# cantwellc/QEC_LDPC

Measured on AMD Instinct MI355X. Metric: syndromes decoded/sec (fixed BP iters), higher is better.
Workload: dtype f32

## Files before the change

### include/qec_ldpc.h

```cpp
#ifndef QEC_LDPC_H
#define QEC_LDPC_H

#include <stddef.h>
#include <stdint.h>

#ifdef __cplusplus
extern "C" {
#endif

#define QEC_LDPC_ABI_VERSION 4

enum {
    QEC_OK = 0,
    QEC_ERR_ARG = -1,
    QEC_ERR_IO = -2,
    QEC_ERR_FORMAT = -3,
    QEC_ERR_UNSUPPORTED = -4,
    QEC_ERR_HIP = -5,
    QEC_ERR_NOMEM = -6
};

enum {
    QEC_SUCCESS = 0,
    QEC_SYNDROME_FAIL_X = 1 << 0,
// ... 62 lines not shown

qec_decoder* qec_decoder_create(const qec_code* code, int device, size_t max_batch);
qec_decoder* qec_decoder_create_engine(const qec_code* code, int device, size_t max_batch, int engine);
int qec_decoder_destroy(qec_decoder* dec);
qec_decoder* qec_decoder_create_multi(const qec_code* code, const int* devices, int ndevices, size_t max_batch);
qec_decoder* qec_decoder_create_multi_engine(const qec_code* code, const int* devices, int ndevices, size_t max_batch,
                                             int engine);
int qec_decoder_num_parts(const qec_decoder* dec);
qec_decoder* qec_decoder_part(qec_decoder* dec, int k);
int qec_decoder_device(const qec_decoder* dec);
enum { QEC_OPT_HARD_PATHS = 1, QEC_OPT_CYCLE_JUMP = 2, QEC_OPT_SCHEDULE = 3, QEC_OPT_SECTOR_SPLIT = 4,
       QEC_OPT_PHASE_STATS = 5, QEC_OPT_TRIAGE = 6, QEC_OPT_LAST_PATH = 7, QEC_OPT_MC_DECODE_TIME = 8,
       QEC_OPT_OSD = 9, QEC_OPT_OSD_ITERATIONS = 10, QEC_OPT_OSD_SECTORS = 11, QEC_OPT_OSD_SWEEP = 12,
       QEC_OPT_OSD_ORDER = 13, QEC_OPT_OSD_CS_SECTORS = 14, QEC_OPT_NEAR_HARD_JUMP = 15, QEC_OPT_OSD_SCORE = 16,
       QEC_OPT_CORRELATED = 17, QEC_OPT_BP_SCHEDULE = 18, QEC_OPT_BP_METHOD = 19, QEC_OPT_MINSUM_SCALE = 20,
       QEC_OPT_MINSUM_WAVE = 21, QEC_OPT_RELAY_WAVE = 22, QEC_OPT_MINSUM_SCHEDULE = 23, QEC_OPT_LIGHT_MEMO = 24 };
enum {
    QEC_PATH_ORDERED = 1,
    QEC_PATH_SECTOR_ORDER = 2,
    QEC_PATH_SPLIT_WAVES = 4,
    QEC_PATH_SECTOR_LAUNCHES = 8,
    QEC_PATH_TRIAGE = 16,
    QEC_PATH_BIT_ROWS = 32,
    QEC_PATH_SPARSE = 64,
    QEC_PATH_RECORDS = 128,
    QEC_PATH_OSD = 256,
    QEC_PATH_CORRELATED = 512,
    QEC_PATH_SERIAL = 1024,
    QEC_PATH_MINSUM = 2048,
    QEC_PATH_RELAY = 4096,
    QEC_PATH_SOFT = 16384,
    QEC_PATH_WAVE = 8192
};
int qec_near_hard_threshold(float pPrime, int R, int L, float* eps0, uint32_t* T);
int qec_decoder_set_option(qec_decoder* dec, int option, int value);
int qec_decoder_get_option(const qec_decoder* dec, int option, int* value);
int qec_decoder_set_priors(qec_decoder* dec, const float* priorX, const float* priorZ);
int qec_decoder_get_priors(const qec_decoder* dec, float* priorX, float* priorZ);
int qec_decoder_get_osd_weights(const qec_decoder* dec, int32_t* wX, int32_t* wZ);
int qec_minsum_llr(float prior, float* llr);
int qec_decoder_get_minsum_llr(const qec_decoder* dec, float* llrX, float* llrZ);
int qec_decoder_set_relay(qec_decoder* dec, const float* gammaX, const float* gammaZ, int legs, int solutions);
int qec_decoder_get_relay(const qec_decoder* dec, float* gammaX, float* gammaZ, int* legs, int* solutions);
int qec_decoder_set_syndrome_priors(qec_decoder* dec, const float* qX, const float* qZ);
int qec_decoder_get_syndrome_priors(const qec_decoder* dec, float* qX, float* qZ);
int qec_correlated_priors(float p, float* c0, float* c1);
int qec_decoder_set_pauli_channel(qec_decoder* dec, const float* pX, const float* pY, const float* pZ);
int qec_decoder_get_pauli_channel(const qec_decoder* dec, float* pX, float* pY, float* pZ);
int qec_decoder_get_conditional_priors(const qec_decoder* dec, float* cZ0, float* cZ1, float* cX0, float* cX1);
// ... 76 lines not shown
```

### qec_ldpc_amd/__init__.py

```python
import ctypes
import os

import numpy as np

_HERE = os.path.dirname(os.path.abspath(__file__))
LIB_PATH = os.path.join(_HERE, "libqecldpc.so")

SUCCESS = 0
SYNDROME_FAIL_X = 1
SYNDROME_FAIL_Z = 2
CONVERGENCE_FAIL_X = 4
CONVERGENCE_FAIL_Z = 8
STOP = {"ref": 0, "fixed": 1, "syndrome": 2}
ENGINE = {"auto": 0, "circulant": 1, "sparse": 2, "cpu": 3}
OPTION = {"hard_paths": 1, "cycle_jump": 2, "schedule": 3, "sector_split": 4, "phase_stats": 5, "triage": 6,
          "last_path": 7, "mc_decode_time": 8, "osd": 9, "osd_iterations": 10, "osd_sectors": 11,
          "osd_sweep": 12, "osd_order": 13, "osd_cs_sectors": 14, "near_hard": 15, "osd_score": 16,
          "correlated": 17, "bp_schedule": 18, "bp_method": 19, "minsum_scale": 20,
          "minsum_wave": 21, "relay_wave": 22, "minsum_schedule": 23, "light_memo": 24}
OPTIONS = OPTION
BP_SCHEDULE = {"flooding": 0, "serial": 1}
BP_METHOD = {"product": 0, "minsum": 1}
MINSUM_SCHEDULE = {"flooding": 0, "layered": 1}
PATH = {"ordered": 1, "sector_order": 2, "split_waves": 4, "sector_launches": 8, "triage": 16, "bit_rows": 32,
        "sparse": 64, "records": 128, "osd": 256, "correlated": 512, "serial": 1024,
        "minsum": 2048, "relay": 4096, "wave": 8192, "soft": 16384}

EXPORTS = (
    "qec_last_error", "qec_abi_version", "qec_build_id",
    "qec_code_load", "qec_code_generate", "qec_code_from_matrices", "qec_code_degrees", "qec_code_layers",
    "qec_code_has_wave_minsum",
    "qec_code_free",
    "qec_code_params", "qec_code_exponents",
    "qec_code_pcm", "qec_code_describe", "qec_code_syndrome", "qec_code_check_logical",
    "qec_code_with_logical", "qec_code_logical_mode", "qec_code_logical_rows", "qec_code_imp",
    "qec_decoder_create", "qec_decoder_create_engine", "qec_decoder_create_multi", "qec_decoder_create_multi_engine",
    "qec_decoder_destroy",
    "qec_decoder_num_parts", "qec_decoder_part", "qec_decoder_device", "qec_decoder_describe",
    "qec_decoder_set_option", "qec_decoder_get_option", "qec_near_hard_threshold",
    "qec_decoder_set_priors", "qec_decoder_get_priors", "qec_decoder_get_osd_weights", "qec_sample_independent_dev",
    "qec_correlated_priors", "qec_minsum_llr", "qec_decoder_get_minsum_llr", "qec_decoder_set_pauli_channel", "qec_decoder_get_pauli_channel",
    "qec_decoder_set_relay", "qec_decoder_get_relay",
    "qec_decoder_set_syndrome_priors", "qec_decoder_get_syndrome_priors",
    "qec_decode_batch_soft", "qec_decode_batch_soft_dev", "qec_flip_syndrome_dev",
    "qec_decoder_get_conditional_priors", "qec_sample_pauli_dev",
    "qec_decode_batch", "qec_decode_batch_dev", "qec_decode_batch_packed", "qec_decode_batch_packed_dev",
    "qec_decode_bits_packed_dev",
    "qec_sample_fixed_weight", "qec_get_statistics",
    "qec_sample_depolarizing_dev", "qec_sample_syndrome_dev", "qec_syndrome_dev", "qec_statistics_dev",
    "qec_statistics_packed_dev", "qec_logical_packed_dev", "qec_pack_decisions_dev",
    "qec_monte_carlo",
    "qec_osd", "qec_osd_dev",
)
LOGICAL = {"file": 0, "reference": 1, "degenerate": 2}
# ... 67 lines not shown
            "qec_code_logical_mode": (i, [vp]),
            "qec_code_logical_rows": (i, [vp, vp]),
            "qec_code_imp": (i, [vp, vp]),
            "qec_decoder_create": (vp, [vp, i, sz]),
            "qec_decoder_create_engine": (vp, [vp, i, sz, i]),
            "qec_decoder_create_multi": (vp, [vp, vp, i, sz]),
            "qec_decoder_create_multi_engine": (vp, [vp, vp, i, sz, i]),
            "qec_decoder_destroy": (i, [vp]),
            "qec_decoder_num_parts": (i, [vp]),
            "qec_decoder_part": (vp, [vp, i]),
            "qec_decoder_device": (i, [vp]),
            "qec_decoder_describe": (i, [vp, ctypes.c_char_p, sz]),
            "qec_decoder_set_option": (i, [vp, i, i]),
            "qec_decoder_get_option": (i, [vp, i, vp]),
            "qec_near_hard_threshold": (i, [f, i, i, vp, vp]),
            "qec_decoder_set_priors": (i, [vp, vp, vp]),
            "qec_decoder_get_priors": (i, [vp, vp, vp]),
            "qec_decoder_get_osd_weights": (i, [vp, vp, vp]),
            "qec_sample_independent_dev": (i, [vp, ctypes.c_uint64, ctypes.c_uint64, sz, vp, vp, vp]),
            "qec_correlated_priors": (i, [f, vp, vp]),
            "qec_minsum_llr": (i, [f, vp]),
            "qec_decoder_get_minsum_llr": (i, [vp, vp, vp]),
            "qec_decoder_set_relay": (i, [vp, vp, vp, i, i]),
            "qec_decoder_get_relay": (i, [vp, vp, vp, vp, vp]),
            "qec_decoder_set_syndrome_priors": (i, [vp, vp, vp]),
            "qec_decoder_get_syndrome_priors": (i, [vp, vp, vp]),
            "qec_decode_batch_soft": (i, [vp, vp, vp, sz, f, i, i, vp, vp, vp, vp, vp, vp, vp]),
            "qec_decode_batch_soft_dev": (i, [vp, vp, vp, sz, f, i, i, vp, vp, vp, vp, vp, vp, vp, vp]),
            "qec_flip_syndrome_dev": (i, [vp, ctypes.c_uint64, ctypes.c_uint64, sz, vp, vp, vp, vp, vp]),
            "qec_decoder_set_pauli_channel": (i, [vp, vp, vp, vp]),
# ... 30 lines not shown
def last_error():
    return lib().qec_last_error().decode()


def build_id():
    return lib().qec_build_id().decode()


def near_hard_threshold(p_prime, R, L):
    eps0, T = ctypes.c_float(0.0), ctypes.c_uint32(0)
    _check(lib().qec_near_hard_threshold(float(np.float32(p_prime)), int(R), int(L), ctypes.byref(eps0), ctypes.byref(T)),
           "qec_near_hard_threshold")
    return float(eps0.value), int(T.value)


def correlated_priors(p):
    c0, c1 = ctypes.c_float(0.0), ctypes.c_float(0.0)
    _check(lib().qec_correlated_priors(float(np.float32(p)), ctypes.byref(c0), ctypes.byref(c1)), "qec_correlated_priors")
    return np.float32(c0.value), np.float32(c1.value)


def has_wave_minsum(code):
    return code.has_wave_minsum()


def minsum_llr(prior):
    llr = ctypes.c_float(0.0)
    _check(lib().qec_minsum_llr(float(np.float32(prior)), ctypes.byref(llr)), "qec_minsum_llr")
    return np.float32(llr.value)

# ... 682 lines not shown
```

### qec_ldpc_amd/csrc/bp_decode.hip

```cpp
#include <hip/hip_runtime.h>

#include <atomic>
#include <cstddef>
#include <cstdint>
#include <cstdio>
#include <cstdlib>
#include <cstring>
#include <type_traits>

#include "qec_device.h"
#include "qec_internal.h"
#include "qec_launch.h"
#include "qec_near.h"
#include "qec_wave.h"

#pragma clang fp contract(off)

namespace qec {

#ifndef QEC_PHASE_STATS
#define QEC_PHASE_STATS 0
#endif
constexpr int kTrackFrom = 2;

// ... 4 lines not shown
    static constexpr int kMinWavesX = MWX_ > 0 ? MWX_ : MINW_;
    static constexpr int kMinWavesZ = MWZ_ > 0 ? MWZ_ : MINW_;
    static constexpr bool kRowBarrier = ROWB_;
    static constexpr int kColGroup = CG_;
    static constexpr int kMinWaves = MINW_;
    static constexpr int kMinWavesSyn = SYNW_ > 0 ? SYNW_ : MINW_;
    static constexpr int kWavesPerBlock = WPB_;
    static constexpr bool kMaskSelect = MASKSEL_;
    static constexpr int kPipeline = PIPE_;
    static constexpr bool kSplit = SPLIT_;
    static constexpr bool kRelabel = RELABEL_;
    static constexpr bool kZeroSkip = ZEROSKIP_;
    static constexpr bool kFastDiv = FASTDIV_;
    static constexpr bool kSaturate = SATURATE_;
    static constexpr bool kAgreeSyn = false;
    static constexpr int kSeqSynWavesX = kMinWavesSyn, kSeqSynWavesZ = kMinWavesSyn;
};

template <class TU>
struct SeqSynTune : TU {
    static constexpr int kSeqSynWavesX = 5 > TU::kMinWavesSyn ? 5 : TU::kMinWavesSyn;
};

template <class TU, int LW, int WPB = 0>
struct ListTune : TU {
    static constexpr int kMinWavesSyn = LW;
    static constexpr int kWavesPerBlock = WPB > 0 ? WPB : TU::kWavesPerBlock;
};

template <class TU, int L>
// ... 57 lines not shown
    uint8_t* rec;
    uint32_t* merge;
    const int32_t* listX;
    const int32_t* listZ;
    const uint32_t* counts;
    int mergeOnly;
    int countStride;
    long long B;
    int P, G, n, mX, mZ;
    int nb, recBytes;
    float errorProbability;
    int maxIter, stop;
    int hardPaths;
    int scaled;
    uint32_t nearT[2];
    alignas(16) float tab0[kMaxTab0];
    uint32_t zs[2];
    const uint16_t* memo;
    int SX[kMaxRL], SZ[kMaxRL];
    int DX[kMaxR], DZ[kMaxR];
    int CX[kMaxL], CZ[kMaxL];
};

struct RuntimeShifts {
    static constexpr bool kStatic = false;
    static constexpr bool kMaskSelect = false;
    static constexpr int kP = 0;
    __device__ static int P(const BpArgs& a) { return a.P; }
    template <int SEC>
    __device__ static const int* table(const BpArgs& a)
// ... 246 lines not shown
        for (int r = 0; r < R; ++r) {
            const int sh = SH::template shift<SEC, L>(et, r, l);
            msg[r][l] = rot<SH>(msg[r][l], ln, sh == 0 ? 0 : P - sh);
        }
}

template <int SEC>
__device__ __forceinline__ uint32_t near_T(const BpArgs&)
{
    static_assert(std::is_standard_layout<BpArgs>::value, "offsetof(BpArgs, nearT)");
    const __attribute__((address_space(4))) uint32_t* k =
        (const __attribute__((address_space(4))) uint32_t*)__builtin_amdgcn_kernarg_segment_ptr();
    asm volatile("" : "+s"(k));
    return k[offsetof(BpArgs, nearT) / sizeof(uint32_t) + SEC];
}

template <int R, int L, int SEC, bool LAST, bool HD, class SH, class TU, int CG = 1, bool SOFT_IN = false,
          bool NEAR = false>
__device__ __forceinline__ uint32_t var_pass(const BpArgs& a, float (&msg)[R][L], const Lane& ln, float pp,
                                             float one_minus_pp, bool& hard, bool& vagree, bool track, bool& near)
{
    static_assert(L % CG == 0, "column groups must tile the L columns");
    const bool hard_in = !SOFT_IN && CG == 1 && hard;
    bool vsame = true;
    uint32_t soft_bits = 0;
    constexpr int F = LAST ? R : R - 1;
    constexpr bool kScalable = TU::kFastDiv && F <= 4;
    const bool scaled = kScalable && a.scaled;
    const float fold0 = scaled ? one_minus_pp * 0x1p32f : one_minus_pp, fold1 = scaled ? pp * 0x1p32f : pp;
    const int P = SH::P(a);
// ... 144 lines not shown
        }
        __builtin_amdgcn_sched_barrier(0);
    }
    if constexpr (TU::kSaturate) {
        const bool forms = track && (a.hardPaths & QEC_HP_FORMS);
        hard = forms && all_live_sh<SH>(soft_bits == 0u, ln.live);
        vagree = hard && all_live_sh<SH>(vsame, ln.live);
        if constexpr (NEAR) {
            const uint32_t nearT = near_T<SEC>(a);
            near = nearT != 0u && forms && all_live_sh<SH>(soft_bits <= nearT && vsame, ln.live);
        }
    }
    return hdmask;
}

template <int R, int L, int SEC, bool HD, class SH>
__device__ __forceinline__ bool var_pass_agree(const BpArgs& a, const float (&msg)[R][L], const Lane& ln,
                                               uint32_t& hdmask)
{
    const int* et = SH::template table<SEC>(a);
    bool same = true;
    uint32_t hd = 0;
#pragma unroll
    for (int l = 0; l < L; ++l) {
        const uint32_t x0 = __float_as_uint(rot<SH>(msg[0][l], ln, SH::template shift<SEC, L>(et, 0, l)));
#pragma unroll
        for (int r = 1; r < R; ++r)
            same &= __float_as_uint(rot<SH>(msg[r][l], ln, SH::template shift<SEC, L>(et, r, l))) == x0;
        if constexpr (HD) hd |= (uint32_t)(x0 == 0x3F800000u) << l;
    }
// ... 62 lines not shown
template <int SEC, int L, class SH>
constexpr bool kRow0Local()
{
    if constexpr (!SH::kStatic) {
        return false;
    } else {
        for (int l = 0; l < L; ++l)
            if (SH::template shift<SEC, L>(nullptr, 0, l) != 0) return false;
        return true;
    }
}

template <int L>
constexpr bool kSkipSeen() { return L < 32; }

template <int R, int L, int SEC, int STOP, bool LAST, class SH, class TU>
__device__ __forceinline__ bool iteration(const BpArgs& a, float (&msg)[R][L], uint32_t sbits, int n, Lane& ln,
                                          float pp, float one_minus_pp, bool& hard, bool& agreed, bool& vagree,
                                          uint32_t& hd_out, uint32_t (&seen)[2], bool& near)
{
    const int P = SH::P(a);
    if constexpr (SH::kMaskSelect) asm volatile("" : "+v"(ln.b0), "+v"(ln.b1));
    constexpr bool HD = STOP == QEC_STOP_SYNDROME;
    uint32_t hdmask = 0;
    agreed = false;
    vagree = false;
    near = false;
    bool unused = false;
    bool var_layout = defer_return<HD, SH>();
    if (TU::kSaturate && hard) {
        check_pass_hard<R, L>(msg, sbits);
        agreed = kAgree<STOP, TU>() && (LAST || R >= 2) && var_pass_agree<R, L, SEC, HD, SH>(a, msg, ln, hdmask);
        if (agreed) {
            vagree = true;
            var_layout = false;
        } else {
            hdmask = var_pass<R, L, SEC, LAST, HD, SH, TU>(a, msg, ln, pp, one_minus_pp, hard, vagree, true, unused);
        }
    } else {
        check_pass<R, L, TU::kRowBarrier>(msg, sbits);
        constexpr int CG = col_group<TU, L>();
        constexpr bool kNear = TU::kSaturate && !LAST && STOP != QEC_STOP_SYNDROME;
        const bool from1 = kNear && near_T<SEC>(a) != 0u;
        const bool track = (LAST || n >= (from1 ? 1 : kTrackFrom)) && (a.hardPaths & QEC_HP_FORMS);
        hdmask = var_pass<R, L, SEC, LAST, HD, SH, TU, CG, true, kNear>(a, msg, ln, pp, one_minus_pp, hard, vagree, track,
                                                                        near);
        if constexpr (kNear) {
            if (near) near = all_live_sh<SH>(lane_parity_ok<R, L>(msg, sbits), ln.live);
        }
    }
    if constexpr (STOP == QEC_STOP_REF) {
        if (n % 10 == 0) return group_all_sh<SH>(lane_converged<R, L>(msg), ln, P);
    } else if constexpr (STOP == QEC_STOP_SYNDROME) {
        hd_out = hdmask;
        const bool same0 = kSkipSeen<L>() && group_all_sh<SH>(hdmask == seen[0], ln, P);
        bool skip = false;
        if constexpr (kSkipSeen<L>()) skip = all_live_sh<SH>(same0 || group_all_sh<SH>(hdmask == seen[1], ln, P), ln.live);
        bool stop = false;
        bool row0_fails = false;
        if constexpr (kRow0Local<SEC, L, SH>()) {
            if (!skip) {
                const bool ok0 = ((__popc(hdmask) ^ sbits) & 1u) == 0u && !(sbits & kNonBinary);
                row0_fails = all_live_sh<SH>(!group_all_sh<SH>(ok0, ln, P), ln.live);
// ... 359 lines not shown
#pragma unroll
        for (int r = 0; r < R; ++r)
#pragma unroll
            for (int l = 0; l < L; ++l) msg[r][l] = pp;
    }

    const float one_minus_pp = 1.0f - pp;
    bool hard = false;
    bool active = in_range;
    int it = 0;
    int n = 0;
    bool in_agree = false, st_agreed = false;
    bool agreed = false, vagree = false;
    bool near = false;
    bool near_done = false;
    int ph_soft = 0, ph_hard = 0, ph_agree = 0, ph_jump = 0;
    uint32_t hd_last = 0;
    bool syn_last = false, hd_valid = false;
    uint32_t seen[2] = {~0u, ~0u};
    bool cv0 = true, msg_built = true;
    unsigned long long hdpat = 0, cvpat = 0;
    if constexpr (STOP == QEC_STOP_SYNDROME && !GO) pattern_masks<R>(tab0, hdpat, cvpat);
    if (N >= 2) {
        uint32_t hd0 = 0;
        const bool stop0 = iteration0<R, L, SEC, STOP, SH, GO>(a, msg, sbits, ln, tab0, hd0, cv0, msg_built, hdpat, cvpat);
        if (active) {
            ++it;
            syn_last = stop0;
            hd_last = hd0;
            hd_valid = true;
            if (STOP == QEC_STOP_SYNDROME && !GO) seen[0] = hd_last;
            if (syn_last) active = false;
            if constexpr (QEC_PHASE_STATS) ph_soft += 1;
        }
        n = 1;
    }
    for (; n < N - 1; ++n) {
        if (!__any(active)) break;
        if (active) {
            ++it;
            const bool was_hard = hard;
            syn_last = iteration<R, L, SEC, STOP, false, SH, TU>(a, msg, sbits, n, ln, pp, one_minus_pp, hard, agreed,
                                                                 vagree, hd_last, seen, near);
            hd_valid = true;
            if (syn_last) active = false;
            if constexpr (QEC_PHASE_STATS) { ph_soft += !was_hard; ph_hard += was_hard && !agreed; ph_agree += agreed; }
            if constexpr (TU::kSaturate) {
                st_agreed = vagree;
                if (agreed && in_agree && active && (a.hardPaths & QEC_HP_CYCLE)) {
                    const int last = cycle_end<STOP>(n, N);
                    if ((last - n) & 1) check_pass_hard<R, L>(msg, sbits);
                    it += last - n;
                    if constexpr (QEC_PHASE_STATS) ph_jump = last - n;
                    active = false;
                    hd_valid = false;
                    n = N;
                }
                in_agree = vagree;
// ... 6 lines not shown
                            for (int l = 0; l < L; ++l) asm volatile("" : "+v"(msg[r][l]));
                        const int last = cycle_end<STOP>(n, N);
                        it += last - n;
                        if constexpr (QEC_PHASE_STATS) ph_jump = last - n;
                        active = false;
                        n = N;
                    }
                }
            }
        }
    }
    if (n == N - 1 && active) {
        ++it;
        const bool was_hard = hard;
        syn_last = iteration<R, L, SEC, STOP, true, SH, TU>(a, msg, sbits, n, ln, pp, one_minus_pp, hard, agreed, vagree,
                                                            hd_last, seen, near);
        hd_valid = true;
        if constexpr (QEC_PHASE_STATS) { ph_soft += !was_hard; ph_hard += was_hard && !agreed; ph_agree += agreed; }
        st_agreed = vagree;
    }

    asm volatile("" : "+v"(sbits));
    const int* et = SH::template table<SEC>(a);
    bool conv, syn_ok;
    uint32_t hdmask = 0;
    if (STOP != QEC_STOP_SYNDROME && TU::kSaturate && all_live(near_done, in_range)) {
#pragma unroll
        for (int l = 0; l < L; ++l)
            hdmask |= (uint32_t)(rot<SH>(msg[0][l], ln, SH::template shift<SEC, L>(et, 0, l)) >= 0.5f) << l;
        conv = true;
        syn_ok = true;
    } else if (STOP == QEC_STOP_SYNDROME && all_live(hd_valid, in_range)) {
        conv = group_all_sh<SH>(__any(in_range && msg_built) ? lane_converged<R, L>(msg) : cv0, ln, P);
        hdmask = hd_last;
        syn_ok = syn_last;
    } else if (TU::kSaturate && all_live(st_agreed, in_range)) {
#pragma unroll
        for (int l = 0; l < L; ++l)
            hdmask |= (uint32_t)(rot<SH>(msg[0][l], ln, SH::template shift<SEC, L>(et, 0, l)) >= 0.5f) << l;
        bool match = true;
#pragma unroll
        for (int r = 0; r < R; ++r) {
            uint32_t x = 0;
#pragma unroll
// ... 184 lines not shown
    const long long slot = grp * G + g;
    const bool in_range = (g < G) && (slot < a.B);
    if (!__any(in_range)) {
        store_tab0();
        return;
    }
    const bool doX = MODE == 3 || (MODE != 4 && (!SPLIT || (wave & 1) == 0));
    const long long pslot = (a.perm_sectors && !doX) ? slot + a.B : slot;
    const uint32_t b = (in_range && a.perm != nullptr) ? (uint32_t)a.perm[pslot] : (uint32_t)slot;
    decode_group<RX, RZ, L, STOP, SH, StopTune<STOP, SH, TU>, MODE>(a, tab0, stage, i, gb, b, in_range, doX, store_tab0);
}

using KernelFn = void (*)(const BpArgs);

using TuneP61 = Tune<5, true, false, true, true, false, true, 2, 1, 4, 1, false, 6, 5>;
struct TuneP61MinReg : TuneP61 {};
using ShiftsP61 = GeneratedShifts<4, 5, 10, 61, 9, 49, TuneP61::kRelabel, TuneP61::kMaskSelect>;
using TuneP7 = Tune<7, true, false, true, true, true, false, 2, 1, 7, 3, false, 0, 0>;
struct TuneP7MinReg : TuneP7 {};
using ShiftsP7 = GeneratedShifts<3, 3, 6, 7, 2, 3, TuneP7::kRelabel, TuneP7::kMaskSelect>;
using ListTuneP61 = ListTune<TuneP61, 4, 16>;
using ListTuneP7 = ListTune<TuneP7MinReg, 5>;
KernelFn p61_minreg_kernel(int stop, bool split);
KernelFn p61_minreg_seq_kernel(int stop, int sec);
KernelFn p7_minreg_kernel(int stop, bool split);
KernelFn p7_minreg_list_kernel();

KernelFn phase_kernel(int P, int stop);

#if defined(QEC_P61_MINREG_TU)
KernelFn p61_minreg_kernel(int stop, bool split)
// ... 248 lines not shown
    }
    a.B = B;
    a.P = c.P;
    a.G = 64 / c.P;
    a.n = c.n; a.mX = c.mX; a.mZ = c.mZ;
    a.nb = (c.n + 7) / 8;
    a.recBytes = rec_stride > 0 ? rec_stride : 2 * a.nb + 1;
    a.errorProbability = errorProbability;
    a.maxIter = maxIter < 0 ? 0 : maxIter;
    a.stop = stop;
    a.hardPaths = hard_ok(2.0f / 3.0f * errorProbability) ? hardPaths & (QEC_HP_FORMS | QEC_HP_CYCLE | QEC_HP_NEAR) : 0;
    a.scaled = scaled_ok(2.0f / 3.0f * errorProbability) ? 1 : 0;
    if ((hardPaths & QEC_HP_FORMS) && (hardPaths & QEC_HP_NEAR) && q == nullptr && stop != QEC_STOP_SYNDROME) {
        a.nearT[0] = near_hard_threshold(2.0f / 3.0f * errorProbability, c.J, c.L).T;
        a.nearT[1] = near_hard_threshold(2.0f / 3.0f * errorProbability, c.K, c.L).T;
    }
    v->fill_tab0(2.0f / 3.0f * errorProbability, a.tab0);
    if (!phase)
        for (int sec = 0; sec < 2; ++sec) a.zs[sec] = v->zero_out[sec](2.0f / 3.0f * errorProbability, a.maxIter, stop);
    a.memo = !phase && v->light_memo && q == nullptr && stop != QEC_STOP_SYNDROME && a.maxIter >= 2 ? memo : nullptr;
    relabel(c.EX.data(), c.J, c.L, c.P, v->relabel, a.SX, a.DX, a.CX);
    relabel(c.EZ.data(), c.K, c.L, c.P, v->relabel, a.SZ, a.DZ, a.CZ);
    const int wavesPerBlock = v->waves_per_block;
    const bool seq = !phase && !split && decode_uses_seq(v, stop, split_opt, B);
    const long long waves = (B + a.G - 1) / a.G * (split ? 2 : 1);
    const long long blocks = (waves + wavesPerBlock - 1) / wavesPerBlock;
    if (blocks > 0x7fffffffLL) return fail(QEC_ERR_ARG, "batch too large for one launch");
    if (seq) {
        if (merge == nullptr) return fail(QEC_ERR_ARG, "bp_decode: sector launches need the merge words");
        a.merge = merge;
// ... 231 lines not shown
```

### qec_ldpc_amd/csrc/capi.cpp

```cpp
#include <hip/hip_runtime.h>

#include <chrono>
#include <cstring>
#include <memory>
#include <new>
#include <stdexcept>
#include <algorithm>
#include <thread>

#include "../../include/HostDeviceArray.h"
#include "qec_internal.h"
#include "qec_near.h"
#include "qec_osd.h"

namespace {
constexpr unsigned kEvNoFence = hipEventDisableSystemFence;
}

namespace qec {
const char* last_error_cstr();
const void* select_variant(const Code& c, std::string& name);
int launch_decode(const void* variant, const Code& c, const uint8_t* sX, const uint8_t* sZ, bool sbits, long long B,
                  float errorProbability, int maxIter, int stop, uint8_t* eX, uint8_t* eZ, uint8_t* flags,
                  uint8_t* rec, int32_t* iters, float* q, int hardPaths, const int32_t* perm, int split,
// ... 113 lines not shown
        return QEC_OK;
    }
};

struct qec_decoder {
    std::shared_ptr<const Code> code;
    int device = 0;
    int engine = QEC_ENGINE_CIRCULANT;
    const void* variant = nullptr;
    void* sparse = nullptr;
    void* cpu = nullptr;
    std::string variant_name;
    int hard_paths = 1;
    int cycle_jump = 1;
    int near_hard = 1;
    int light_memo = 1;
    DeviceArray<uint16_t> memo_tab;
    DeviceArray<uint8_t> memo_ws;
    bool memo_valid = false;
    uint32_t memo_key[3] = {0, 0, 0};
    int schedule = 1;
    int sector_split = 1;
    int phase_stats = 0;
    int triage = 1;
    int last_path = 0;
    int mc_time = 1;
    int osd = 0;
    int osd_iters = 3;
    int osd_sweep = 0;
    unsigned long long osd_sectors = 0;
// ... 496 lines not shown
        text += " [relay: " + wave_relay_name(*d->code) + "]";
    if (d->has_syn) text += " [soft syndrome]";
    std::snprintf(buf, len, "%s", text.c_str());
    return QEC_OK;
}

int qec_near_hard_threshold(float pPrime, int R, int L, float* eps0, uint32_t* T)
{
    if (!eps0 || !T) return fail(QEC_ERR_ARG, "qec_near_hard_threshold: bad argument");
    const NearHard t = near_hard_threshold(pPrime, R, L);
    *eps0 = t.eps0;
    *T = t.T;
    return QEC_OK;
}

static int set_wave_option(qec_decoder* d, int value, int& field, const std::string& name, const char* what,
                           const char* alone, const void* (*select)(const Code&))
{
    const std::string who = "qec_decoder_set_option: " + name;
    if (value != 0 && value != 1) return fail(QEC_ERR_ARG, who + " is 0 (the sparse-graph kernels) or 1 (the wave kernels)");
    if (value && d->parts.empty()) {
        if (d->cpu)
            return fail(QEC_ERR_UNSUPPORTED,
                        who + " = 1 chooses GPU kernels; the CPU engine has one " + what + " implementation");
        if (d->engine != QEC_ENGINE_SPARSE)
            return fail(QEC_ERR_UNSUPPORTED,
                        who + " = 1 is a kernel choice of a sparse-engine handle, which alone " + alone +
                            "; create the decoder with QEC_ENGINE_SPARSE (engine \"sparse\")");
        if (!select(*d->code))
            return fail(QEC_ERR_UNSUPPORTED,
// ... 4 lines not shown
    field = value;
    return QEC_OK;
}

int qec_decoder_set_option(qec_decoder* d, int option, int value)
{
    if (!d) return fail(QEC_ERR_ARG, "qec_decoder_set_option: null decoder");
    for (qec_decoder* p : d->parts) {
        const int rc = qec_decoder_set_option(p, option, value);
        if (rc) return rc;
    }
    switch (option) {
    case QEC_OPT_HARD_PATHS: d->hard_paths = value != 0; return QEC_OK;
    case QEC_OPT_CYCLE_JUMP: d->cycle_jump = value != 0; return QEC_OK;
    case QEC_OPT_NEAR_HARD_JUMP: d->near_hard = value != 0; return QEC_OK;
    case QEC_OPT_LIGHT_MEMO: d->light_memo = value != 0; return QEC_OK;
    case QEC_OPT_SCHEDULE:
        if (value < 0 || value > 4) return fail(QEC_ERR_ARG, "qec_decoder_set_option: QEC_OPT_SCHEDULE is 0 .. 4");
        d->schedule = value;
        return QEC_OK;
    case QEC_OPT_SECTOR_SPLIT:
        if (value < 0 || value > 3) return fail(QEC_ERR_ARG, "qec_decoder_set_option: QEC_OPT_SECTOR_SPLIT is 0 .. 3");
        d->sector_split = value;
        return QEC_OK;
    case QEC_OPT_PHASE_STATS:
        if (value && (!d->variant || !decode_has_phase_stats(d->variant, QEC_STOP_FIXED)))
            return fail(QEC_ERR_UNSUPPORTED, "qec_decoder_set_option: QEC_OPT_PHASE_STATS needs a shipped code's kernels");
        d->phase_stats = value != 0;
        return QEC_OK;
    case QEC_OPT_TRIAGE:
// ... 464 lines not shown
    if (!d) return fail(QEC_ERR_ARG, "qec_decoder_get_osd_weights: null decoder");
    if (!d->has_priors) return 0;
    const int n = d->code->n;
    if (wX) std::memcpy(wX, d->osw.data(), n * sizeof(int32_t));
    if (wZ) std::memcpy(wZ, d->osw.data() + n, n * sizeof(int32_t));
    return 1;
}

int qec_decoder_get_option(const qec_decoder* d, int option, int* value)
{
    if (!d || !value) return fail(QEC_ERR_ARG, "qec_decoder_get_option: bad argument");
    switch (option) {
    case QEC_OPT_HARD_PATHS: *value = d->hard_paths; return QEC_OK;
    case QEC_OPT_CYCLE_JUMP: *value = d->cycle_jump; return QEC_OK;
    case QEC_OPT_NEAR_HARD_JUMP: *value = d->near_hard; return QEC_OK;
    case QEC_OPT_LIGHT_MEMO: *value = d->light_memo; return QEC_OK;
    case QEC_OPT_SCHEDULE: *value = d->schedule; return QEC_OK;
    case QEC_OPT_SECTOR_SPLIT: *value = d->sector_split; return QEC_OK;
    case QEC_OPT_PHASE_STATS: *value = d->phase_stats; return QEC_OK;
    case QEC_OPT_TRIAGE: *value = d->triage; return QEC_OK;
    case QEC_OPT_LAST_PATH: *value = d->parts.empty() ? d->last_path : d->parts[0]->last_path; return QEC_OK;
    case QEC_OPT_MC_DECODE_TIME: *value = d->mc_time; return QEC_OK;
    case QEC_OPT_OSD: *value = d->osd; return QEC_OK;
    case QEC_OPT_OSD_ITERATIONS: *value = d->osd_iters; return QEC_OK;
    case QEC_OPT_OSD_SWEEP: *value = d->osd_sweep; return QEC_OK;
    case QEC_OPT_OSD_SECTORS: {
        unsigned long long t = d->osd_sectors;
        for (const qec_decoder* p : d->parts) t += p->osd_sectors;
        *value = (int)std::min<unsigned long long>(t, 0x7FFFFFFFull);
        return QEC_OK;
// ... 17 lines not shown
    }
}

}

namespace {

constexpr long long kScheduleMinBatch = 4096;
constexpr long long kScheduleMaxSingle = 1LL << 19;
constexpr float kScheduleSyndromeMinP = 0.004f;
constexpr float kTriageMaxP = 0.01f;
constexpr long long kSplitOrderedMinBatch = 1LL << 19;

int hard_path_bits(const qec_decoder* d)
{
    return (d->hard_paths ? (QEC_HP_FORMS | (d->cycle_jump ? QEC_HP_CYCLE : 0) | (d->near_hard ? QEC_HP_NEAR : 0)) : 0) |
           (d->phase_stats ? QEC_HP_PHASE : 0);
}

bool triage_on(const qec_decoder* d, float p)
{
    return !d->phase_stats && (d->triage == 2 || ((d->triage == 1 || d->triage == 3) && p <= kTriageMaxP));
}

int dispatch_decode(qec_decoder* d, const uint8_t* sX, const uint8_t* sZ, long long B, float p, int maxIter, int stop,
                    uint8_t* eX, uint8_t* eZ, uint8_t* flags, uint8_t* rec, int32_t* iters, float* q, hipStream_t st,
                    bool sbits = false, int rec_stride = 0, uint8_t* fX = nullptr, uint8_t* fZ = nullptr)
{
    if (B <= 0) return QEC_OK;
    const Code& c = *d->code;
    int rc = ws_acquire(d, st);
// ... 1101 lines not shown
```

### qec_ldpc_amd/csrc/qec_internal.h

```cpp
#pragma once
#include <cstdint>
#include <string>
#include <vector>

#include "../../include/qec_ldpc.h"

namespace qec {

enum { QEC_HP_FORMS = 1, QEC_HP_CYCLE = 2, QEC_HP_PHASE = 4 ,
       QEC_HP_NEAR = 8  };
enum { QEC_ORDER_GLOBAL = 0, QEC_ORDER_LOCAL = 1, QEC_ORDER_ONE_LAUNCH = 2 };

void set_error(const std::string& msg);
int fail(int status, const std::string& msg);

struct Code {
    int J = 0, K = 0, L = 0, P = 0, sigma = 0, tau = 0;
    int n = 0, mX = 0, mZ = 0;
    std::vector<uint8_t> pcmX, pcmZ;
    std::vector<uint8_t> imp;
    int logical_mode = 0;
    bool is_qc = false;
    bool general = false;
    int D = 0, dvX = 0, dvZ = 0, k = 0;
    int stride() const { return general ? D : L; }
// ... 96 lines not shown
```

### qec_ldpc_amd/csrc/qec_near.h

```cpp
#pragma once
#include <cmath>
#include <cstdint>
#include <cstring>

namespace qec {

struct NearHard {
    float eps0;
    uint32_t T;
};

inline NearHard near_hard_threshold(float pp, int R, int L)
{
    NearHard out{0.0f, 0u};
    if (!(pp > 0.0f && pp <= 0.5f) || R < 2 || L < 2 || L > 32) return out;
    const double odds = (1.0 - (double)pp) / (double)pp;
    for (int k = 8; k <= 20; ++k) {
        const double e = std::ldexp(1.0, -k);
        const double d = (L - 1) * e + 0x1p-20;
        if (!(d < 0.5)) continue;
        const double ratio = d / (1.0 - d);
        double x = 2.0 * odds;
        for (int f = 0; f < R - 1; ++f) x *= ratio;
        if (!(x * (1.0 + 0x1p-40) <= e)) continue;
        out.eps0 = (float)e;
        const float v = (float)(e - e * e);
        std::memcpy(&out.T, &v, sizeof v);
        out.T -= 1u;
        return out;
    }
    return out;
}

}
```

Baseline: 281.2 million.

## Add near-hard probe that decides hard bits from bit-pattern margins before var pass

Adds a cheaper variable-node probe that compares float bit patterns of the extrinsic products against a threshold K derived from the near-hard epsilon. When every live lane clears the margin and its syndrome checks out, the full var_pass is skipped and the hard decisions are kept for the final output. The probe is on by default through a new option, but only for the P61 tune. It adds per-iteration probe work and extra state, which is wasted whenever the probe fails and var_pass still runs.

```diff
diff --git a/include/qec_ldpc.h b/include/qec_ldpc.h
--- a/include/qec_ldpc.h
+++ b/include/qec_ldpc.h
@@ -100,7 +100,8 @@
        QEC_OPT_OSD = 9, QEC_OPT_OSD_ITERATIONS = 10, QEC_OPT_OSD_SECTORS = 11, QEC_OPT_OSD_SWEEP = 12,
        QEC_OPT_OSD_ORDER = 13, QEC_OPT_OSD_CS_SECTORS = 14, QEC_OPT_NEAR_HARD_JUMP = 15, QEC_OPT_OSD_SCORE = 16,
        QEC_OPT_CORRELATED = 17, QEC_OPT_BP_SCHEDULE = 18, QEC_OPT_BP_METHOD = 19, QEC_OPT_MINSUM_SCALE = 20,
-       QEC_OPT_MINSUM_WAVE = 21, QEC_OPT_RELAY_WAVE = 22, QEC_OPT_MINSUM_SCHEDULE = 23, QEC_OPT_LIGHT_MEMO = 24 };
+       QEC_OPT_MINSUM_WAVE = 21, QEC_OPT_RELAY_WAVE = 22, QEC_OPT_MINSUM_SCHEDULE = 23, QEC_OPT_LIGHT_MEMO = 24,
+       QEC_OPT_NEAR_PROBE = 25 };
 enum {
     QEC_PATH_ORDERED = 1,
     QEC_PATH_SECTOR_ORDER = 2,
@@ -119,6 +120,7 @@
     QEC_PATH_WAVE = 8192
 };
 int qec_near_hard_threshold(float pPrime, int R, int L, float* eps0, uint32_t* T);
+int qec_near_probe(float t0, float t1, float eps0, int* side);
 int qec_decoder_set_option(qec_decoder* dec, int option, int value);
 int qec_decoder_get_option(const qec_decoder* dec, int option, int* value);
 int qec_decoder_set_priors(qec_decoder* dec, const float* priorX, const float* priorZ);
diff --git a/qec_ldpc_amd/__init__.py b/qec_ldpc_amd/__init__.py
--- a/qec_ldpc_amd/__init__.py
+++ b/qec_ldpc_amd/__init__.py
@@ -17,7 +17,8 @@
           "last_path": 7, "mc_decode_time": 8, "osd": 9, "osd_iterations": 10, "osd_sectors": 11,
           "osd_sweep": 12, "osd_order": 13, "osd_cs_sectors": 14, "near_hard": 15, "osd_score": 16,
           "correlated": 17, "bp_schedule": 18, "bp_method": 19, "minsum_scale": 20,
-          "minsum_wave": 21, "relay_wave": 22, "minsum_schedule": 23, "light_memo": 24}
+          "minsum_wave": 21, "relay_wave": 22, "minsum_schedule": 23, "light_memo": 24,
+          "near_probe": 25}
 OPTIONS = OPTION
 BP_SCHEDULE = {"flooding": 0, "serial": 1}
 BP_METHOD = {"product": 0, "minsum": 1}
@@ -37,7 +38,7 @@
     "qec_decoder_create", "qec_decoder_create_engine", "qec_decoder_create_multi", "qec_decoder_create_multi_engine",
     "qec_decoder_destroy",
     "qec_decoder_num_parts", "qec_decoder_part", "qec_decoder_device", "qec_decoder_describe",
-    "qec_decoder_set_option", "qec_decoder_get_option", "qec_near_hard_threshold",
+    "qec_decoder_set_option", "qec_decoder_get_option", "qec_near_hard_threshold", "qec_near_probe",
     "qec_decoder_set_priors", "qec_decoder_get_priors", "qec_decoder_get_osd_weights", "qec_sample_independent_dev",
     "qec_correlated_priors", "qec_minsum_llr", "qec_decoder_get_minsum_llr", "qec_decoder_set_pauli_channel", "qec_decoder_get_pauli_channel",
     "qec_decoder_set_relay", "qec_decoder_get_relay",
@@ -135,6 +136,7 @@
             "qec_decoder_set_option": (i, [vp, i, i]),
             "qec_decoder_get_option": (i, [vp, i, vp]),
             "qec_near_hard_threshold": (i, [f, i, i, vp, vp]),
+            "qec_near_probe": (i, [f, f, f, vp]),
             "qec_decoder_set_priors": (i, [vp, vp, vp]),
             "qec_decoder_get_priors": (i, [vp, vp, vp]),
             "qec_decoder_get_osd_weights": (i, [vp, vp, vp]),
@@ -195,6 +197,12 @@
     return float(eps0.value), int(T.value)
 
 
+def near_probe(t0, t1, eps0):
+    side = ctypes.c_int(0)
+    ok = lib().qec_near_probe(float(np.float32(t0)), float(np.float32(t1)), float(np.float32(eps0)), ctypes.byref(side))
+    return bool(ok), int(side.value)
+
+
 def correlated_priors(p):
     c0, c1 = ctypes.c_float(0.0), ctypes.c_float(0.0)
     _check(lib().qec_correlated_priors(float(np.float32(p)), ctypes.byref(c0), ctypes.byref(c1)), "qec_correlated_priors")
diff --git a/qec_ldpc_amd/csrc/bp_decode.hip b/qec_ldpc_amd/csrc/bp_decode.hip
--- a/qec_ldpc_amd/csrc/bp_decode.hip
+++ b/qec_ldpc_amd/csrc/bp_decode.hip
@@ -42,6 +42,7 @@
     static constexpr bool kFastDiv = FASTDIV_;
     static constexpr bool kSaturate = SATURATE_;
     static constexpr bool kAgreeSyn = false;
+    static constexpr bool kNearProbe = false;
     static constexpr int kSeqSynWavesX = kMinWavesSyn, kSeqSynWavesZ = kMinWavesSyn;
 };
 
@@ -129,6 +130,7 @@
     int hardPaths;
     int scaled;
     uint32_t nearT[2];
+    uint32_t nearK[2];
     alignas(16) float tab0[kMaxTab0];
     uint32_t zs[2];
     const uint16_t* memo;
@@ -405,6 +407,14 @@
     asm volatile("" : "+s"(k));
     return k[offsetof(BpArgs, nearT) / sizeof(uint32_t) + SEC];
 }
+template <int SEC>
+__device__ __forceinline__ uint32_t near_K(const BpArgs&)
+{
+    const __attribute__((address_space(4))) uint32_t* k =
+        (const __attribute__((address_space(4))) uint32_t*)__builtin_amdgcn_kernarg_segment_ptr();
+    asm volatile("" : "+s"(k));
+    return k[offsetof(BpArgs, nearK) / sizeof(uint32_t) + SEC];
+}
 
 template <int R, int L, int SEC, bool LAST, bool HD, class SH, class TU, int CG = 1, bool SOFT_IN = false,
           bool NEAR = false>
@@ -579,6 +589,49 @@
     return hdmask;
 }
 
+template <int R, int L, int SEC, class SH, class TU, int CG>
+__device__ __forceinline__ bool var_probe(const BpArgs& a, const float (&msg)[R][L], const Lane& ln, float pp,
+                                          float one_minus_pp, uint32_t K, uint32_t& hd_near)
+{
+    static_assert(L % CG == 0, "column groups must tile the L columns");
+    constexpr bool kScalable = TU::kFastDiv && R - 1 <= 4;
+    const bool scaled = kScalable && a.scaled;
+    const float fold0 = scaled ? one_minus_pp * 0x1p32f : one_minus_pp, fold1 = scaled ? pp * 0x1p32f : pp;
+    const int* et = SH::template table<SEC>(a);
+    int32_t margin = 0x7FFFFFFF;
+    uint32_t top = 0, hd = 0;
+#pragma unroll
+    for (int l0 = 0; l0 < L; l0 += CG) {
+#pragma unroll
+        for (int c = 0; c < CG; ++c) {
+            const int l = l0 + c;
+            float gv[R];
+#pragma unroll
+            for (int r = 0; r < R; ++r) gv[r] = rot<SH>(msg[r][l], ln, SH::template shift<SEC, L>(et, r, l));
+            float bv[R];
+#pragma unroll
+            for (int r = 0; r < R; ++r) bv[r] = 1.0f - gv[r];
+            NearProbeVar pv;
+            float pre0 = fold0, pre1 = fold1;
+#pragma unroll
+            for (int j = 0; j < R; ++j) {
+                float t0 = pre0, t1 = pre1;
+#pragma unroll
+                for (int k = j + 1; k < R; ++k) { t0 = t0 * bv[k]; t1 = t1 * gv[k]; }
+                pv.add(__float_as_uint(t0), __float_as_uint(t1), top);
+                if (j + 1 < R) { pre0 = pre0 * bv[j]; pre1 = pre1 * gv[j]; }
+            }
+            margin = min(margin, pv.margin());
+            hd |= (uint32_t)pv.side() << l;
+            asm volatile("" : "+v"(hd));
+        }
+        if (l0 == 0 && !all_live_sh<SH>(margin >= (int32_t)K && top < kNearProbeTop, ln.live)) return false;
+        __builtin_amdgcn_sched_barrier(0);
+    }
+    hd_near = hd;
+    return all_live_sh<SH>(margin >= (int32_t)K && top < kNearProbeTop, ln.live);
+}
+
 template <int R, int L, int SEC, bool HD, class SH>
 __device__ __forceinline__ bool var_pass_agree(const BpArgs& a, const float (&msg)[R][L], const Lane& ln,
                                                uint32_t& hdmask)
@@ -671,10 +724,19 @@
 template <int L>
 constexpr bool kSkipSeen() { return L < 32; }
 
+template <int STOP, class SH, class TU>
+constexpr bool kNearProbe()
+{
+    if constexpr (SH::kStatic)
+        return TU::kNearProbe && TU::kSaturate && !QEC_PHASE_STATS && STOP != QEC_STOP_SYNDROME && 2 * SH::kP > 64;
+    else
+        return false;
+}
+
 template <int R, int L, int SEC, int STOP, bool LAST, class SH, class TU>
 __device__ __forceinline__ bool iteration(const BpArgs& a, float (&msg)[R][L], uint32_t sbits, int n, Lane& ln,
                                           float pp, float one_minus_pp, bool& hard, bool& agreed, bool& vagree,
-                                          uint32_t& hd_out, uint32_t (&seen)[2], bool& near)
+                                          uint32_t& hd_out, uint32_t (&seen)[2], bool& near, uint32_t& hd_near)
 {
     const int P = SH::P(a);
     if constexpr (SH::kMaskSelect) asm volatile("" : "+v"(ln.b0), "+v"(ln.b1));
@@ -700,10 +762,44 @@
         constexpr bool kNear = TU::kSaturate && !LAST && STOP != QEC_STOP_SYNDROME;
         const bool from1 = kNear && near_T<SEC>(a) != 0u;
         const bool track = (LAST || n >= (from1 ? 1 : kTrackFrom)) && (a.hardPaths & QEC_HP_FORMS);
-        hdmask = var_pass<R, L, SEC, LAST, HD, SH, TU, CG, true, kNear>(a, msg, ln, pp, one_minus_pp, hard, vagree, track,
-                                                                        near);
-        if constexpr (kNear) {
-            if (near) near = all_live_sh<SH>(lane_parity_ok<R, L>(msg, sbits), ln.live);
+        bool probed = false;
+        if constexpr (kNear && kNearProbe<STOP, SH, TU>()) {
+            const uint32_t K = near_K<SEC>(a);
+            if (band(band(track, K != 0u), STOP != QEC_STOP_REF || n % 10 != 0)) {
+                uint32_t hdn = 0;
+                if (var_probe<R, L, SEC, SH, TU, CG>(a, msg, ln, pp, one_minus_pp, K, hdn)) {
+                    if constexpr (SH::kMaskSelect) asm volatile("" : "+v"(ln.b0), "+v"(ln.b1));
+                    probed = all_live_sh<SH>(lane_syndrome_ok<R, L, SEC, SH>(a, hdn, sbits, ln), ln.live);
+                    if (probed) {
+                        near = true;
+                        hd_near = hdn;
+                    }
+                }
+            }
+        }
+        if (!probed) {
+            if constexpr (kNear && kNearProbe<STOP, SH, TU>() && SH::kMaskSelect) asm volatile("" : "+v"(ln.b0), "+v"(ln.b1));
+            if constexpr (kNear && kNearProbe<STOP, SH, TU>()) {
+#pragma unroll
+                for (int r = 0; r < R; ++r)
+#pragma unroll
+                    for (int l = 0; l < L; ++l) asm volatile("" : "+v"(msg[r][l]));
+            }
+            hdmask = var_pass<R, L, SEC, LAST, HD, SH, TU, CG, true, kNear>(a, msg, ln, pp, one_minus_pp, hard, vagree,
+                                                                            track, near);
+            if constexpr (kNear) {
+                if (near) near = all_live_sh<SH>(lane_parity_ok<R, L>(msg, sbits), ln.live);
+                if constexpr (kNearProbe<STOP, SH, TU>()) {
+                    if (near) {
+                        const int* et = SH::template table<SEC>(a);
+                        uint32_t hdn = 0;
+#pragma unroll
+                        for (int l = 0; l < L; ++l)
+                            hdn |= (uint32_t)(rot<SH>(msg[0][l], ln, SH::template shift<SEC, L>(et, 0, l)) >= 0.5f) << l;
+                        hd_near = hdn;
+                    }
+                }
+            }
         }
     }
     if constexpr (STOP == QEC_STOP_REF) {
@@ -1093,6 +1189,7 @@
     bool agreed = false, vagree = false;
     bool near = false;
     bool near_done = false;
+    uint32_t hd_near;
     int ph_soft = 0, ph_hard = 0, ph_agree = 0, ph_jump = 0;
     uint32_t hd_last = 0;
     bool syn_last = false, hd_valid = false;
@@ -1120,7 +1217,7 @@
             ++it;
             const bool was_hard = hard;
             syn_last = iteration<R, L, SEC, STOP, false, SH, TU>(a, msg, sbits, n, ln, pp, one_minus_pp, hard, agreed,
-                                                                 vagree, hd_last, seen, near);
+                                                                 vagree, hd_last, seen, near, hd_near);
             hd_valid = true;
             if (syn_last) active = false;
             if constexpr (QEC_PHASE_STATS) { ph_soft += !was_hard; ph_hard += was_hard && !agreed; ph_agree += agreed; }
@@ -1157,7 +1254,7 @@
         ++it;
         const bool was_hard = hard;
         syn_last = iteration<R, L, SEC, STOP, true, SH, TU>(a, msg, sbits, n, ln, pp, one_minus_pp, hard, agreed, vagree,
-                                                            hd_last, seen, near);
+                                                            hd_last, seen, near, hd_near);
         hd_valid = true;
         if constexpr (QEC_PHASE_STATS) { ph_soft += !was_hard; ph_hard += was_hard && !agreed; ph_agree += agreed; }
         st_agreed = vagree;
@@ -1168,9 +1265,13 @@
     bool conv, syn_ok;
     uint32_t hdmask = 0;
     if (STOP != QEC_STOP_SYNDROME && TU::kSaturate && all_live(near_done, in_range)) {
-#pragma unroll
-        for (int l = 0; l < L; ++l)
-            hdmask |= (uint32_t)(rot<SH>(msg[0][l], ln, SH::template shift<SEC, L>(et, 0, l)) >= 0.5f) << l;
+        if constexpr (kNearProbe<STOP, SH, TU>()) {
+            hdmask = hd_near;
+        } else {
+#pragma unroll
+            for (int l = 0; l < L; ++l)
+                hdmask |= (uint32_t)(rot<SH>(msg[0][l], ln, SH::template shift<SEC, L>(et, 0, l)) >= 0.5f) << l;
+        }
         conv = true;
         syn_ok = true;
     } else if (STOP == QEC_STOP_SYNDROME && all_live(hd_valid, in_range)) {
@@ -1385,7 +1486,9 @@
 using KernelFn = void (*)(const BpArgs);
 
 using TuneP61 = Tune<5, true, false, true, true, false, true, 2, 1, 4, 1, false, 6, 5>;
-struct TuneP61MinReg : TuneP61 {};
+struct TuneP61MinReg : TuneP61 {
+    static constexpr bool kNearProbe = true;
+};
 using ShiftsP61 = GeneratedShifts<4, 5, 10, 61, 9, 49, TuneP61::kRelabel, TuneP61::kMaskSelect>;
 using TuneP7 = Tune<7, true, false, true, true, true, false, 2, 1, 7, 3, false, 0, 0>;
 struct TuneP7MinReg : TuneP7 {};
@@ -1664,6 +1767,10 @@
     if ((hardPaths & QEC_HP_FORMS) && (hardPaths & QEC_HP_NEAR) && q == nullptr && stop != QEC_STOP_SYNDROME) {
         a.nearT[0] = near_hard_threshold(2.0f / 3.0f * errorProbability, c.J, c.L).T;
         a.nearT[1] = near_hard_threshold(2.0f / 3.0f * errorProbability, c.K, c.L).T;
+        if (hardPaths & QEC_HP_NEAR_PROBE) {
+            a.nearK[0] = near_probe_scale(near_hard_threshold(2.0f / 3.0f * errorProbability, c.J, c.L).eps0);
+            a.nearK[1] = near_probe_scale(near_hard_threshold(2.0f / 3.0f * errorProbability, c.K, c.L).eps0);
+        }
     }
     v->fill_tab0(2.0f / 3.0f * errorProbability, a.tab0);
     if (!phase)
diff --git a/qec_ldpc_amd/csrc/capi.cpp b/qec_ldpc_amd/csrc/capi.cpp
--- a/qec_ldpc_amd/csrc/capi.cpp
+++ b/qec_ldpc_amd/csrc/capi.cpp
@@ -151,6 +151,7 @@
     int hard_paths = 1;
     int cycle_jump = 1;
     int near_hard = 1;
+    int near_probe = 1;
     int light_memo = 1;
     DeviceArray<uint16_t> memo_tab;
     DeviceArray<uint8_t> memo_ws;
@@ -677,6 +678,14 @@
     return QEC_OK;
 }
 
+int qec_near_probe(float t0, float t1, float eps0, int* side)
+{
+    int s = 0;
+    const bool ok = near_probe(t0, t1, eps0, s);
+    if (side) *side = s;
+    return ok ? 1 : 0;
+}
+
 static int set_wave_option(qec_decoder* d, int value, int& field, const std::string& name, const char* what,
                            const char* alone, const void* (*select)(const Code&))
 {
@@ -711,6 +720,7 @@
     case QEC_OPT_HARD_PATHS: d->hard_paths = value != 0; return QEC_OK;
     case QEC_OPT_CYCLE_JUMP: d->cycle_jump = value != 0; return QEC_OK;
     case QEC_OPT_NEAR_HARD_JUMP: d->near_hard = value != 0; return QEC_OK;
+    case QEC_OPT_NEAR_PROBE: d->near_probe = value != 0; return QEC_OK;
     case QEC_OPT_LIGHT_MEMO: d->light_memo = value != 0; return QEC_OK;
     case QEC_OPT_SCHEDULE:
         if (value < 0 || value > 4) return fail(QEC_ERR_ARG, "qec_decoder_set_option: QEC_OPT_SCHEDULE is 0 .. 4");
@@ -1205,6 +1215,7 @@
     case QEC_OPT_HARD_PATHS: *value = d->hard_paths; return QEC_OK;
     case QEC_OPT_CYCLE_JUMP: *value = d->cycle_jump; return QEC_OK;
     case QEC_OPT_NEAR_HARD_JUMP: *value = d->near_hard; return QEC_OK;
+    case QEC_OPT_NEAR_PROBE: *value = d->near_probe; return QEC_OK;
     case QEC_OPT_LIGHT_MEMO: *value = d->light_memo; return QEC_OK;
     case QEC_OPT_SCHEDULE: *value = d->schedule; return QEC_OK;
     case QEC_OPT_SECTOR_SPLIT: *value = d->sector_split; return QEC_OK;
@@ -1252,7 +1263,7 @@
 
 int hard_path_bits(const qec_decoder* d)
 {
-    return (d->hard_paths ? (QEC_HP_FORMS | (d->cycle_jump ? QEC_HP_CYCLE : 0) | (d->near_hard ? QEC_HP_NEAR : 0)) : 0) |
+    return (d->hard_paths ? (QEC_HP_FORMS | (d->cycle_jump ? QEC_HP_CYCLE : 0) | (d->near_hard ? QEC_HP_NEAR | (d->near_probe ? QEC_HP_NEAR_PROBE : 0) : 0)) : 0) |
            (d->phase_stats ? QEC_HP_PHASE : 0);
 }
 
diff --git a/qec_ldpc_amd/csrc/qec_internal.h b/qec_ldpc_amd/csrc/qec_internal.h
--- a/qec_ldpc_amd/csrc/qec_internal.h
+++ b/qec_ldpc_amd/csrc/qec_internal.h
@@ -8,7 +8,8 @@
 namespace qec {
 
 enum { QEC_HP_FORMS = 1, QEC_HP_CYCLE = 2, QEC_HP_PHASE = 4 ,
-       QEC_HP_NEAR = 8  };
+       QEC_HP_NEAR = 8 ,
+       QEC_HP_NEAR_PROBE = 16  };
 enum { QEC_ORDER_GLOBAL = 0, QEC_ORDER_LOCAL = 1, QEC_ORDER_ONE_LAUNCH = 2 };
 
 void set_error(const std::string& msg);
diff --git a/qec_ldpc_amd/csrc/qec_near.h b/qec_ldpc_amd/csrc/qec_near.h
--- a/qec_ldpc_amd/csrc/qec_near.h
+++ b/qec_ldpc_amd/csrc/qec_near.h
@@ -32,4 +32,47 @@
     return out;
 }
 
+inline uint32_t near_probe_scale(float eps0)
+{
+    int e = 0;
+    if (!(eps0 > 0.0f) || std::frexp(eps0, &e) != 0.5f) return 0u;
+    const int k = 1 - e;
+    return k >= 8 && k <= 20 ? (uint32_t)(k + 1) << 23 : 0u;
 }
+constexpr uint32_t kNearProbeTop = 0x7F000000u;
+#if defined(__HIPCC__)
+#define QEC_NEAR_HD __host__ __device__ __forceinline__
+#else
+#define QEC_NEAR_HD inline
+#endif
+struct NearProbeVar {
+    int32_t mn = 0x7FFFFFFF, mx = -0x7FFFFFFF - 1;
+    QEC_NEAR_HD void add(uint32_t b0, uint32_t b1, uint32_t& top)
+    {
+        const int32_t d = (int32_t)(b1 - b0);
+        mn = d < mn ? d : mn;
+        mx = d > mx ? d : mx;
+        top = top > b0 ? top : b0;
+        top = top > b1 ? top : b1;
+    }
+    QEC_NEAR_HD int32_t margin() const
+    {
+        const int32_t neg = (int32_t)(0u - (uint32_t)mx);
+        return mn > neg ? mn : neg;
+    }
+    QEC_NEAR_HD bool side() const { return mn > 0; }
+};
+#undef QEC_NEAR_HD
+inline bool near_probe(float t0, float t1, float eps0, int& side)
+{
+    uint32_t b0, b1, top = 0u;
+    std::memcpy(&b0, &t0, sizeof t0);
+    std::memcpy(&b1, &t1, sizeof t1);
+    const uint32_t K = near_probe_scale(eps0);
+    NearProbeVar v;
+    v.add(b0, b1, top);
+    side = v.side();
+    return K != 0u && top < kNearProbeTop && v.margin() >= (int32_t)K;
+}
+
+}
```

Measured after the change: 311.8 million, median of 6. 1.11x the previous value.
